# ACMMM2021-Anonymous/video-graph-ssl

Measured on AMD Instinct MI355X. Metric: pretrain_clips_per_sec, higher is better.
Workload: dtype bf16x6 (fp32 tensors; conv products as 6 bf16 MFMAs on hi/mid/lo splits = fp32-grade, fp32 accumulate; everything else fp32)

## Files before the change

__graft_entry__.py:

```python
import importlib
import os
import subprocess
import sys

ROOT = os.path.dirname(os.path.abspath(__file__))
if ROOT not in sys.path:
    sys.path.insert(0, ROOT)
CSRC = os.path.join(ROOT, 'video-graph-ssl_amd', 'csrc')
SOURCES = ['conv3d', 'conv3d_halo', 'conv3d_stem', 'conv3d_pw', 'conv3d_wgrad', 'conv3d_wgrad_ts', 'conv3d_wgrad_stem', 'bn', 'pool', 'misc', 'infonce', 'graph', 'input', 'augment', 'retrieval']


def _hipcc():
    for c in (os.environ.get('HIPCC'), '/opt/rocm/bin/hipcc', 'hipcc'):
        if c and (os.path.isabs(c) and os.path.exists(c) or not os.path.isabs(c)):
            return c
    raise RuntimeError('hipcc not found')


def build(force=False):
    out = os.path.join(ROOT, 'video-graph-ssl_amd', 'libgca_hip.so')
    srcs = [os.path.join(CSRC, s + '.hip') for s in SOURCES]
    deps = srcs + [os.path.join(CSRC, h) for h in ('gca_common.h', 'conv_common.h', 'conv_igemm_host.h', 'conv_halo.h')] + [
                   os.path.join(ROOT, 'include', 'gca_hip.h')]
    stale = force or not os.path.exists(out) or any(os.path.getmtime(d) > os.path.getmtime(out) for d in deps)
    if stale:
        hipcc = _hipcc()
        flags = ['-O3', '--offload-arch=gfx950', '-fPIC', '-std=c++17']
        procs = []
        for s in SOURCES:
            cmd = [hipcc] + flags + ['-c', os.path.join(CSRC, s + '.hip'), '-o', os.path.join(CSRC, s + '.o')]
            procs.append((s, subprocess.Popen(cmd, stdout=subprocess.PIPE, stderr=subprocess.STDOUT)))
        for s, p in procs:
            log = p.communicate()[0].decode()
            if p.returncode != 0:
                raise RuntimeError('hipcc failed on %s.hip:\n%s' % (s, log))
        subprocess.check_call([hipcc, '--offload-arch=gfx950', '-shared', '-fPIC', '-o', out] +
                              [os.path.join(CSRC, s + '.o') for s in SOURCES])
# ... 28 lines not shown
```

include/gca_hip.h:

```cpp
#ifndef GCA_HIP_H
#define GCA_HIP_H

#include <stdint.h>

#ifdef __cplusplus
extern "C" {
#endif

#define GCA_OK 0
#define GCA_EINVAL (-1)
#define GCA_ELAUNCH (-2)

int gca_version(void);

int gca_conv_halo_occupancy(int tm, int tn, int math, int64_t lds_bytes);

int gca_set_conv_math(int mode);
int gca_get_conv_math(void);

typedef struct {
  int32_t N, C, D, H, W;
  int32_t K;
  int32_t kd, kh, kw;
  int32_t sd, sh, sw;
// ... 91 lines not shown
               const float* scale, const float* shift, void* ws, int act_f16, void* stream);
int64_t gca_bn_bwd_consts_elems(int64_t C);
int gca_bn_bwd_sums(const void* dz_in, const void* x, const float* gamma, const float* save_mean, const float* save_invstd,
                    int relu, int64_t N, int64_t C, int64_t SP, float* dgamma, float* dbeta, int64_t z_batch_stride ,
                    const float* scale, const float* shift, float* consts, void* ws, int act_f16, void* stream);

typedef struct {
  int32_t N, C, D, H, W;
  int32_t kd, kh, kw, sd, sh, sw, pd, ph, pw;
  int32_t OD, OH, OW;
} gca_pool_geom;
int gca_maxpool3d_fwd(const gca_pool_geom* g, const void* x, void* y, int32_t* argmax, const float* scale,
                      const float* shift, int act_f16, void* stream);
int gca_maxpool3d_bwd(const gca_pool_geom* g, const void* dy, const int32_t* argmax, void* dx,
                      int accumulate, int act_f16, void* stream);
int gca_avgpool3d_fwd(const gca_pool_geom* g, const float* x, float* y, void* stream);
int gca_avgpool3d_bwd(const gca_pool_geom* g, const float* dy, float* dx, int accumulate, void* stream);
int gca_wavgpool_fwd(const void* x, const float* wt, float norm, int64_t NC, int64_t D, int64_t HW,
                     float* y, int x_f16, void* stream);
int gca_wavgpool_bwd(const float* dy, const float* wt, float norm, int64_t NC, int64_t D, int64_t HW,
                     void* dx, int x_f16, void* stream);

int gca_relu_fwd(const float* x, int64_t n, float* y, void* stream);
int gca_relu_bwd(const float* dy, const float* y, int64_t n, float* dx, void* stream);
int gca_l2norm_fwd(const float* x, int64_t rows, int64_t dim, float eps, float* y, float* inv_norm, void* stream);
int gca_l2norm_bwd(const float* dy, const float* y, const float* inv_norm, int64_t rows, int64_t dim,
                   float* dx, void* stream);
int gca_negcos_fwd_bwd(const float* p, const float* z, int64_t rows, int64_t dim, float scale,
                       float* loss, int accumulate, float* dp, void* stream);

// ... 68 lines not shown
```

video-graph-ssl_amd/_hip.py:

```python
import ctypes as C
import os

import torch

_HERE = os.path.dirname(os.path.abspath(__file__))
LIB_PATH = os.environ.get('GCA_LIB_PATH') or os.path.join(_HERE, 'libgca_hip.so')


class HipLibraryMissing(RuntimeError):
    pass


if not os.path.exists(LIB_PATH):
    raise HipLibraryMissing(
        'libgca_hip.so is not built (%s). Run ./build_hip.sh or __graft_entry__.build(); there is no '
        'CPU fallback for the product path.' % LIB_PATH)
lib = C.CDLL(LIB_PATH)

c_i32, c_i64, c_f32, c_f64, c_vp = C.c_int32, C.c_int64, C.c_float, C.c_double, C.c_void_p


class ConvGeom(C.Structure):
    _fields_ = [(n, c_i32) for n in ('N', 'C', 'D', 'H', 'W', 'K', 'kd', 'kh', 'kw', 'sd', 'sh', 'sw',
                                     'pd', 'ph', 'pw', 'OD', 'OH', 'OW')] + [('x_batch_stride', c_i64)] + \
# ... 30 lines not shown
    'gca_conv_wgrad': (c_i32, [_GP, c_vp, c_vp, c_vp, c_vp, c_i32, c_vp, c_vp]),
    'gca_bias_grad': (c_i32, [c_vp, c_i64, c_i64, c_i64, c_vp, c_i32, c_vp]),
    'gca_bn_stats': (c_i32, [c_vp, c_i64, c_i64, c_i64, c_vp, c_vp, c_vp, c_i32, c_vp]),
    'gca_bn_stats_parts': (c_i64, [c_i64, c_i64, c_i64]),
    'gca_bn_finalize': (c_i32, [c_vp, c_vp, c_i64, c_i64, c_f64, c_vp, c_vp, c_f32, c_f32, c_vp, c_vp, c_vp,
                                c_vp, c_vp, c_vp, c_vp, c_vp]),
    'gca_bn_train_fwd': (c_i32, [c_vp, c_vp, c_i64, c_i64, c_f64, c_vp, c_vp, c_f32, c_f32, c_vp, c_vp, c_vp,
                                 c_vp, c_vp, c_vp, c_vp, c_vp, c_vp, c_i32, c_i64, c_i64, c_vp, c_i64, c_i32, c_vp]),
    'gca_bn_fold_eval': (c_i32, [c_vp, c_vp, c_vp, c_vp, c_f32, c_i64, c_vp, c_vp, c_vp]),
    'gca_bn_apply': (c_i32, [c_vp, c_vp, c_vp, c_vp, c_i32, c_i64, c_i64, c_i64, c_vp, c_i64, c_i32, c_vp]),
    'gca_bn_bwd_ws_bytes': (c_i64, [c_i64, c_i64, c_i64]),
    'gca_bn_bwd': (c_i32, [c_vp, c_vp, c_vp, c_vp, c_vp, c_vp, c_i32, c_i64, c_i64, c_i64, c_vp, c_vp, c_vp,
                           c_vp, c_i32, c_i64, c_vp, c_vp, c_vp, c_i32, c_vp]),
    'gca_maxpool3d_fwd': (c_i32, [_PP, c_vp, c_vp, c_vp, c_vp, c_vp, c_i32, c_vp]),
    'gca_maxpool3d_bwd': (c_i32, [_PP, c_vp, c_vp, c_vp, c_i32, c_i32, c_vp]),
    'gca_avgpool3d_fwd': (c_i32, [_PP, c_vp, c_vp, c_vp]),
    'gca_avgpool3d_bwd': (c_i32, [_PP, c_vp, c_vp, c_i32, c_vp]),
    'gca_wavgpool_fwd': (c_i32, [c_vp, c_vp, c_f32, c_i64, c_i64, c_i64, c_vp, c_i32, c_vp]),
    'gca_wavgpool_bwd': (c_i32, [c_vp, c_vp, c_f32, c_i64, c_i64, c_i64, c_vp, c_i32, c_vp]),
    'gca_relu_fwd': (c_i32, [c_vp, c_i64, c_vp, c_vp]),
    'gca_relu_bwd': (c_i32, [c_vp, c_vp, c_i64, c_vp, c_vp]),
    'gca_l2norm_fwd': (c_i32, [c_vp, c_i64, c_i64, c_f32, c_vp, c_vp, c_vp]),
    'gca_l2norm_bwd': (c_i32, [c_vp, c_vp, c_vp, c_i64, c_i64, c_vp, c_vp]),
    'gca_negcos_fwd_bwd': (c_i32, [c_vp, c_vp, c_i64, c_i64, c_f32, c_vp, c_i32, c_vp, c_vp]),
    'gca_infonce_ws_bytes': (c_i64, [c_i64, c_i64]),
    'gca_moco_logits_fwd': (c_i32, [c_vp, c_vp, c_vp, c_i64, c_i64, c_i64, c_f32, c_vp, c_vp, c_vp, c_vp, c_vp, c_vp, c_vp]),
    'gca_nce_softmax_loss_fwd': (c_i32, [c_vp, c_i64, c_i64, c_vp, c_vp, c_vp, c_vp]),
    'gca_nce_softmax_loss_bwd': (c_i32, [c_vp, c_vp, c_i64, c_i64, c_vp, c_f32, c_vp, c_vp]),
    'gca_moco_logits_bwd': (c_i32, [c_vp, c_vp, c_vp, c_vp, c_f32, c_vp, c_vp, c_i64, c_i64, c_i64, c_f32,
                                    c_i64, c_vp, c_i64, c_vp, c_vp, c_vp, c_vp]),
# ... 95 lines not shown
```

video-graph-ssl_amd/csrc/bn.hip:

```cpp
#include "gca_common.h"

namespace {

constexpr int STAT_CHUNK = 8192;
constexpr int MAX_PARTS = 256;
constexpr long long BN_SMALL_ELEMS = 32768;

__host__ __device__ inline long long stats_parts(long long N, long long C, long long SP) {
  long long p = (N * SP + STAT_CHUNK - 1) / STAT_CHUNK;
  if (p < 1) p = 1;
  if (p > MAX_PARTS) p = MAX_PARTS;
  return p;
}

template <typename T, int MODE, int VEC>
__global__ __launch_bounds__(256) void bn_reduce_kernel(
    const T* __restrict__ a, const T* __restrict__ z, const T* __restrict__ x,
    const float* __restrict__ mean, const float* __restrict__ invstd, int relu,
    long long N, long long C, long long SP, long long zs, int P, float* __restrict__ out0,
    float* __restrict__ out1, const float* __restrict__ scale, const float* __restrict__ shift) {
  typedef gca_act<T> A_;
  __shared__ double sh[4];
  const int c = blockIdx.y, part = blockIdx.x;
  const float rsc = relu == 2 ? scale[c] : 0.f, rsf = relu == 2 ? shift[c] : 0.f;
// ... 494 lines not shown
      if (VEC == 4) {
        A_::st4(dx + xi[u], make_float4(ov[0], ov[VEC > 1 ? 1 : 0], ov[VEC > 2 ? 2 : 0], ov[VEC > 3 ? 3 : 0]));
        if (dres) {
          float4 r = make_float4(dv[u][0], dv[u][VEC > 1 ? 1 : 0], dv[u][VEC > 2 ? 2 : 0], dv[u][VEC > 3 ? 3 : 0]);
          if (dres_acc) { r.x += ro[u].x; r.y += ro[u].y; r.z += ro[u].z; r.w += ro[u].w; }
          A_::st4(dres + xi[u], r);
        }
      } else {
        A_::st(dx + xi[u], ov[0]);
        if (dres) A_::st(dres + xi[u], dres_acc ? ro[u].x + dv[u][0] : dv[u][0]);
      }
    }
  }
}

inline unsigned ew_grid(long long total, int vec) {
  long long b = gca_ceil_div(total, 256LL * vec);
  if (b > 8192) b = 8192;
  if (b < 1) b = 1;
  return (unsigned)b;
}

}

extern "C" int gca_bn_finalize(const float* stat_sum, const float* stat_sq, int64_t P, int64_t C, double count,
                               const float* gamma, const float* beta, float eps, float momentum,
                               float* running_mean, float* running_var, int64_t* num_batches_tracked,
                               float* save_mean, float* save_invstd, float* scale, float* shift, void* stream);

template <typename T>
// ... 122 lines not shown
                         const float* scale, const float* shift, float* consts, void* ws, void* stream) {
  if (!dz_in || !x || !save_mean || !save_invstd || !consts || !ws || N <= 0 || C <= 0 || SP <= 0) return GCA_EINVAL;
  if ((relu != 0 && relu != 2) || (relu == 2 && (!scale || !shift))) return GCA_EINVAL;
  if (z_batch_stride != 0 && z_batch_stride < C * SP) return GCA_EINVAL;
  if (C > 0x7fffffffLL - 32) return GCA_EINVAL;
  const long long zs = z_batch_stride ? z_batch_stride : C * SP;
  const int Cp = (int)gca_bn_consts_stride(C);
  hipStream_t st = (hipStream_t)stream;
  bn_bwd_sums_launch<T>(dz_in, dz_in, x, gamma, save_mean, save_invstd, relu, N, C, SP, zs, dgamma, dbeta, scale, shift, ws,
                        consts, (long long)Cp, st);
  hipLaunchKernelGGL(bn_bwd_consts_kernel, dim3((unsigned)gca_ceil_div(Cp, 256)), dim3(256), 0, st, save_mean, save_invstd,
                     scale, shift, relu, (int)C, Cp, consts);
  return gca_launch_status();
}

extern "C" {

int64_t gca_bn_stats_parts(int64_t N, int64_t C, int64_t SP) { return stats_parts(N, C, SP); }


int gca_bn_finalize(const float* stat_sum, const float* stat_sq, int64_t P, int64_t C, double count,
                    const float* gamma, const float* beta, float eps, float momentum,
                    float* running_mean, float* running_var, int64_t* num_batches_tracked,
                    float* save_mean, float* save_invstd, float* scale, float* shift, void* stream) {
  if (!stat_sum || !stat_sq || P <= 0 || C <= 0 || count <= 0 || !scale || !shift) return GCA_EINVAL;
  hipLaunchKernelGGL(bn_finalize_kernel, dim3((unsigned)C), dim3(256), 0, (hipStream_t)stream, stat_sum, stat_sq,
                     (long long)P, count, gamma, beta, eps, momentum, running_mean, running_var, save_mean,
                     save_invstd, scale, shift, (long long*)num_batches_tracked);
  return gca_launch_status();
}
// ... 74 lines not shown
int64_t gca_bn_bwd_consts_elems(int64_t C) {
  if (C <= 0 || C > 0x7fffffffLL - 32) return GCA_EINVAL;
  return GCA_BN_BWD_CONST_ROWS * gca_bn_consts_stride(C);
}

int gca_bn_bwd_sums(const void* dz_in, const void* x, const float* gamma, const float* save_mean, const float* save_invstd,
                    int relu, int64_t N, int64_t C, int64_t SP, float* dgamma, float* dbeta, int64_t z_batch_stride,
                    const float* scale, const float* shift, float* consts, void* ws, int act_f16, void* stream) {
  if (act_f16)
    return bn_bwd_sums_t<gca_half>((const gca_half*)dz_in, (const gca_half*)x, gamma, save_mean, save_invstd, relu, N, C, SP,
                                   dgamma, dbeta, z_batch_stride, scale, shift, consts, ws, stream);
  return bn_bwd_sums_t<float>((const float*)dz_in, (const float*)x, gamma, save_mean, save_invstd, relu, N, C, SP, dgamma, dbeta,
                              z_batch_stride, scale, shift, consts, ws, stream);
}

}
```

video-graph-ssl_amd/csrc/pool.hip:

```cpp
#include "gca_common.h"
#include <math.h>
#include <cstdlib>

namespace {

struct PoolMagic {
  gca_magic osp, ohw, ow;
  gca_magic sp, hw, w;
  gca_magic sd, sh, sw;
  gca_magic c;
};

template <typename T, int KD, int KH, int KW>
__global__ __launch_bounds__(256) void maxpool3d_fwd_kernel(gca_pool_geom g, PoolMagic q, const T* __restrict__ x,
                                                            T* __restrict__ y, int* __restrict__ argmax,
                                                            unsigned total, const float* __restrict__ scale,
                                                            const float* __restrict__ shift) {
  const unsigned i = blockIdx.x * 256u + threadIdx.x;
  if (i >= total) return;
  const unsigned plane = gca_fdiv(i, q.osp), o = i - plane * q.osp.d;
  float sc = 1.f, sf = 0.f;
  if (scale) { const unsigned c = plane - gca_fdiv(plane, q.c) * q.c.d; sc = scale[c]; sf = shift[c]; }
#define GCA_POOL_VAL(v) (scale ? fmaxf((v) * sc + sf, 0.f) : (v))
  const int od = (int)gca_fdiv(o, q.ohw), r = (int)(o - (unsigned)od * q.ohw.d);
// ... 136 lines not shown
        }
#pragma unroll
    for (int e = 0; e < CD * CH * CW; ++e) acc += (okv[e] && am[e] == s) ? gv[e] : 0.f;
  } else {
    for (int od = od_lo; od <= od_hi; ++od)
      for (int oh = oh_lo; oh <= oh_hi; ++oh)
        for (int ow = ow_lo; ow <= ow_hi; ++ow) {
          const long long o = obase + (long long)od * OHW + oh * g.OW + ow;
          if (argmax[o] == s) acc += (float)dy[o];
        }
  }
  dx[i] = (T)(accumulate ? (float)dx[i] + acc : acc);
}

template <typename T>
__global__ __launch_bounds__(256) void maxpool3d_bwd_brick333s2_kernel(gca_pool_geom g, gca_magic msp, gca_magic mhw, gca_magic mw,
                                                                       const T* __restrict__ dy, const int* __restrict__ argmax,
                                                                       T* __restrict__ dx, unsigned nbricks, int accumulate) {
  const unsigned t = blockIdx.x * 256u + threadIdx.x;
  if (t >= nbricks) return;
  const unsigned plane = gca_fdiv(t, msp), sidx = t - plane * msp.d;
  const int n = (int)gca_fdiv(sidx, mhw), r = (int)(sidx - (unsigned)n * mhw.d);
  const int m = (int)gca_fdiv((unsigned)r, mw), j = r - m * (int)mw.d;
  const bool vd1 = n + 1 < g.OD, vh1 = m + 1 < g.OH, vw2 = 2 * j + 2 < g.OW;
  const unsigned o00 = ((plane * (unsigned)g.OD + (unsigned)n) * (unsigned)g.OH + (unsigned)m) * (unsigned)g.OW + 2u * (unsigned)j;
  const unsigned step_d = vd1 ? (unsigned)(g.OH * g.OW) : 0u, step_h = vh1 ? (unsigned)g.OW : 0u, step_w = vw2 ? 2u : 1u;
  int2 a01[4];
  int a2[4];
  float g0[4], g1[4], g2[4];
#pragma unroll
  for (int c = 0; c < 4; ++c) {
    const unsigned o = o00 + ((c & 2) ? step_d : 0u) + ((c & 1) ? step_h : 0u);
    a01[c] = *reinterpret_cast<const int2*>(argmax + o);
    a2[c] = argmax[o + step_w];
    if (sizeof(T) == 4) {
      const float2 v = *reinterpret_cast<const float2*>(dy + o);
      g0[c] = v.x; g1[c] = v.y;
    } else {
      typedef _Float16 h2 __attribute__((ext_vector_type(2)));
      const h2 v = *reinterpret_cast<const h2*>(dy + o);
      g0[c] = (float)v.x; g1[c] = (float)v.y;
    }
    g2[c] = (float)dy[o + step_w];
  }
  if (!vw2) { a2[0] = a2[1] = a2[2] = a2[3] = -1; }
  if (!vd1) { a01[2] = a01[3] = make_int2(-1, -1); a2[2] = a2[3] = -1; }
  if (!vh1) { a01[1] = a01[3] = make_int2(-1, -1); a2[1] = a2[3] = -1; }
  const unsigned plane_base = plane * (unsigned)(g.D * g.H * g.W);
#pragma unroll
  for (int dd = 0; dd < 2; ++dd)
#pragma unroll
    for (int hh = 0; hh < 2; ++hh) {
      const int d = 2 * n + dd, h = 2 * m + hh;
      if (d >= g.D || h >= g.H) continue;
      const int s0 = (d * g.H + h) * g.W + 4 * j;
      float acc[4] = {0.f, 0.f, 0.f, 0.f};
#pragma unroll
      for (int cd = 0; cd <= dd; ++cd)
#pragma unroll
        for (int ch = 0; ch <= hh; ++ch) {
          const int c = 2 * cd + ch;
          acc[0] += a01[c].x == s0 ? g0[c] : 0.f;
          acc[1] += a01[c].x == s0 + 1 ? g0[c] : 0.f;
          acc[1] += a01[c].y == s0 + 1 ? g1[c] : 0.f;
          acc[2] += a01[c].y == s0 + 2 ? g1[c] : 0.f;
          acc[3] += a01[c].y == s0 + 3 ? g1[c] : 0.f;
          acc[3] += a2[c] == s0 + 3 ? g2[c] : 0.f;
        }
      T* out = dx + (plane_base + (unsigned)s0);
      if (accumulate) {
        const float4 o = gca_act<T>::ld4(out);
        acc[0] += o.x; acc[1] += o.y; acc[2] += o.z; acc[3] += o.w;
      }
      gca_act<T>::st4(out, make_float4(acc[0], acc[1], acc[2], acc[3]));
    }
}

template <typename T>
__global__ __launch_bounds__(256) void wavgpool_fwd_kernel(const T* __restrict__ x, const float* __restrict__ wt,
                                                           float norm, long long NC, int D, int HW,
                                                           float* __restrict__ y) {
  const long long p = (long long)blockIdx.x * 4 + (threadIdx.x >> 6);
  if (p >= NC) return;
// ... 8 lines not shown
  s = gca_wave_sum(s);
  if (lane == 0) y[p] = s * norm;
}

template <typename T>
__global__ __launch_bounds__(256) void wavgpool_bwd_kernel(const float* __restrict__ dy, const float* __restrict__ wt,
                                                           float norm, long long total, int D, int HW,
                                                           T* __restrict__ dx) {
  const long long i = (long long)blockIdx.x * 256 + threadIdx.x;
  if (i >= total) return;
  const long long p = i / ((long long)D * HW);
  const int d = (int)((i / HW) % D);
  dx[i] = (T)(dy[p] * norm * (wt ? wt[d] : 1.f));
}

inline bool pool_ok(const gca_pool_geom* g) {
  if (!g || g->N <= 0 || g->C <= 0 || g->D <= 0 || g->H <= 0 || g->W <= 0) return false;
  if (g->kd <= 0 || g->kh <= 0 || g->kw <= 0 || g->sd <= 0 || g->sh <= 0 || g->sw <= 0) return false;
  if (g->pd < 0 || g->ph < 0 || g->pw < 0 || 2 * g->pd > g->kd || 2 * g->ph > g->kh || 2 * g->pw > g->kw) return false;
  if (g->OD != (g->D + 2 * g->pd - g->kd) / g->sd + 1 || g->OH != (g->H + 2 * g->ph - g->kh) / g->sh + 1 ||
      g->OW != (g->W + 2 * g->pw - g->kw) / g->sw + 1)
    return false;
  return g->OD > 0 && g->OH > 0 && g->OW > 0;
}


__global__ __launch_bounds__(256) void avgpool3d_fwd_kernel(gca_pool_geom g, PoolMagic q, const float* __restrict__ x,
                                                            float* __restrict__ y, unsigned total) {
  const unsigned i = blockIdx.x * 256u + threadIdx.x;
  if (i >= total) return;
  const unsigned plane = gca_fdiv(i, q.osp), o = i - plane * q.osp.d;
  const int od = (int)gca_fdiv(o, q.ohw), r = (int)(o - (unsigned)od * q.ohw.d);
  const int oh = (int)gca_fdiv((unsigned)r, q.ow), ow = r - oh * g.OW;
  const float* xp = x + (long long)plane * ((long long)g.D * g.H * g.W);
  float s = 0.f;
  for (int a = 0; a < g.kd; ++a)
    for (int b = 0; b < g.kh; ++b)
      for (int c = 0; c < g.kw; ++c) s += xp[((od * g.kd + a) * g.H + oh * g.kh + b) * g.W + ow * g.kw + c];
  y[i] = s / (float)(g.kd * g.kh * g.kw);
}
__global__ __launch_bounds__(256) void avgpool3d_bwd_kernel(gca_pool_geom g, PoolMagic q, const float* __restrict__ dy,
// ... 20 lines not shown
}

static PoolMagic pool_magic(const gca_pool_geom* g) {
  PoolMagic q;
  q.osp = gca_make_magic((unsigned)(g->OD * g->OH * g->OW)); q.ohw = gca_make_magic((unsigned)(g->OH * g->OW));
  q.ow = gca_make_magic((unsigned)g->OW);
  q.sp = gca_make_magic((unsigned)(g->D * g->H * g->W)); q.hw = gca_make_magic((unsigned)(g->H * g->W));
  q.w = gca_make_magic((unsigned)g->W);
  q.c = gca_make_magic((unsigned)g->C);
  q.sd = gca_make_magic((unsigned)g->sd); q.sh = gca_make_magic((unsigned)g->sh); q.sw = gca_make_magic((unsigned)g->sw);
  return q;
}

int gca_maxpool3d_fwd(const gca_pool_geom* g, const void* x, void* y, int32_t* argmax, const float* scale,
                      const float* shift, int act_f16, void* stream) {
  if (!pool_ok(g) || !x || !y || ((scale == nullptr) != (shift == nullptr))) return GCA_EINVAL;
  const long long total = (long long)g->N * g->C * g->OD * g->OH * g->OW;
  if (total >= (1LL << 31) || (long long)g->D * g->H * g->W >= (1LL << 31)) return GCA_EINVAL;
  const PoolMagic q = pool_magic(g);
  const dim3 grid((unsigned)gca_ceil_div(total, 256));
  hipStream_t st = (hipStream_t)stream;
#define GCA_POOL_FWD(KD, KH, KW)                                                                                              \
  do {                                                                                                                      \
    if (act_f16)                                                                                                            \
      hipLaunchKernelGGL((maxpool3d_fwd_kernel<gca_half, KD, KH, KW>), grid, dim3(256), 0, st, *g, q, (const gca_half*)x,   \
                         (gca_half*)y, argmax, (unsigned)total, scale, shift);                                              \
    else                                                                                                                    \
      hipLaunchKernelGGL((maxpool3d_fwd_kernel<float, KD, KH, KW>), grid, dim3(256), 0, st, *g, q, (const float*)x,         \
                         (float*)y, argmax, (unsigned)total, scale, shift);                                                 \
  } while (0)
  const size_t esz = act_f16 ? 2 : 4;
  if (g->kd == 3 && g->kh == 3 && g->kw == 3 && g->sd == 2 && g->sh == 2 && g->sw == 2 && g->pd == 1 && g->ph == 1 && g->pw == 1 &&
      g->W % 4 == 0 && ((uintptr_t)x % (4 * esz)) == 0 && ((uintptr_t)y % (2 * esz)) == 0 && ((uintptr_t)argmax % 8) == 0 &&
      pool_tiled_on()) {
    const unsigned npairs = (unsigned)(total / 2);
    const gca_magic psp = gca_make_magic((unsigned)(g->OD * g->OH * (g->OW / 2))), phw = gca_make_magic((unsigned)(g->OH * (g->OW / 2))),
                    pw2 = gca_make_magic((unsigned)(g->OW / 2));
    const dim3 pgrid((unsigned)gca_ceil_div((long long)npairs, 256));
    if (act_f16)
      hipLaunchKernelGGL(maxpool3d_fwd_pair333s2_kernel<gca_half>, pgrid, dim3(256), 0, st, *g, psp, phw, pw2, q.c, (const gca_half*)x,
                         (gca_half*)y, argmax, npairs, scale, shift);
    else
      hipLaunchKernelGGL(maxpool3d_fwd_pair333s2_kernel<float>, pgrid, dim3(256), 0, st, *g, psp, phw, pw2, q.c, (const float*)x,
                         (float*)y, argmax, npairs, scale, shift);
    return gca_launch_status();
  }
  if (g->kd == 3 && g->kh == 3 && g->kw == 3) GCA_POOL_FWD(3, 3, 3);
  else if (g->kd == 1 && g->kh == 3 && g->kw == 3) GCA_POOL_FWD(1, 3, 3);
  else if (g->kd == 2 && g->kh == 2 && g->kw == 2) GCA_POOL_FWD(2, 2, 2);
  else GCA_POOL_FWD(0, 0, 0);
#undef GCA_POOL_FWD
  return gca_launch_status();
}

int gca_maxpool3d_bwd(const gca_pool_geom* g, const void* dy, const int32_t* argmax, void* dx,
                      int accumulate, int act_f16, void* stream) {
  if (!pool_ok(g) || !dy || !argmax || !dx) return GCA_EINVAL;
  const long long total = (long long)g->N * g->C * g->D * g->H * g->W;
  if (total >= (1LL << 31)) return GCA_EINVAL;
  const PoolMagic q = pool_magic(g);
  const dim3 grid((unsigned)gca_ceil_div(total, 256));
  hipStream_t st = (hipStream_t)stream;
  const int cd = (int)gca_ceil_div(g->kd, g->sd), ch = (int)gca_ceil_div(g->kh, g->sh), cw = (int)gca_ceil_div(g->kw, g->sw);
#define GCA_POOL_BWD(CD, CH, CW)                                                                                             \
  do {                                                                                                                     \
    if (act_f16)                                                                                                           \
      hipLaunchKernelGGL((maxpool3d_bwd_kernel<gca_half, CD, CH, CW>), grid, dim3(256), 0, st, *g, q, (const gca_half*)dy, \
                         argmax, (gca_half*)dx, (unsigned)total, accumulate ? 1 : 0);                                      \
    else                                                                                                                   \
      hipLaunchKernelGGL((maxpool3d_bwd_kernel<float, CD, CH, CW>), grid, dim3(256), 0, st, *g, q, (const float*)dy,       \
                         argmax, (float*)dx, (unsigned)total, accumulate ? 1 : 0);                                         \
  } while (0)
  if (g->kd == 3 && g->kh == 3 && g->kw == 3 && g->sd == 2 && g->sh == 2 && g->sw == 2 && g->pd == 1 && g->ph == 1 && g->pw == 1 &&
      g->W % 4 == 0 && ((uintptr_t)dx % (act_f16 ? 8 : 16)) == 0 && ((uintptr_t)dy % (act_f16 ? 4 : 8)) == 0 &&
      ((uintptr_t)argmax % 8) == 0 && pool_tiled_on()) {
    const int d2 = (g->D + 1) / 2, h2 = (g->H + 1) / 2, w4 = g->W / 4;
    const unsigned nbricks = (unsigned)((long long)g->N * g->C * d2 * h2 * w4);
    const gca_magic msp = gca_make_magic((unsigned)(d2 * h2 * w4)), mhw = gca_make_magic((unsigned)(h2 * w4)),
                    mw = gca_make_magic((unsigned)w4);
    const dim3 bgrid((unsigned)gca_ceil_div((long long)nbricks, 256));
    if (act_f16)
      hipLaunchKernelGGL(maxpool3d_bwd_brick333s2_kernel<gca_half>, bgrid, dim3(256), 0, st, *g, msp, mhw, mw, (const gca_half*)dy,
                         argmax, (gca_half*)dx, nbricks, accumulate ? 1 : 0);
    else
      hipLaunchKernelGGL(maxpool3d_bwd_brick333s2_kernel<float>, bgrid, dim3(256), 0, st, *g, msp, mhw, mw, (const float*)dy,
                         argmax, (float*)dx, nbricks, accumulate ? 1 : 0);
    return gca_launch_status();
  }
  if (cd == 2 && ch == 2 && cw == 2) GCA_POOL_BWD(2, 2, 2);
  else if (cd == 1 && ch == 2 && cw == 2) GCA_POOL_BWD(1, 2, 2);
  else if (cd == 3 && ch == 3 && cw == 3) GCA_POOL_BWD(3, 3, 3);
  else if (cd == 1 && ch == 1 && cw == 1) GCA_POOL_BWD(1, 1, 1);
  else GCA_POOL_BWD(0, 0, 0);
#undef GCA_POOL_BWD
  return gca_launch_status();
}

static bool avgpool_ok(const gca_pool_geom* g) {
  return pool_ok(g) && g->sd == g->kd && g->sh == g->kh && g->sw == g->kw && g->pd == 0 && g->ph == 0 && g->pw == 0;
}
int gca_avgpool3d_fwd(const gca_pool_geom* g, const float* x, float* y, void* stream) {
  if (!avgpool_ok(g) || !x || !y) return GCA_EINVAL;
  const long long total = (long long)g->N * g->C * g->OD * g->OH * g->OW;
  if (total >= (1LL << 31) || (long long)g->D * g->H * g->W >= (1LL << 31)) return GCA_EINVAL;
  hipLaunchKernelGGL(avgpool3d_fwd_kernel, dim3((unsigned)gca_ceil_div(total, 256)), dim3(256), 0, (hipStream_t)stream, *g,
                     pool_magic(g), x, y, (unsigned)total);
  return gca_launch_status();
}
int gca_avgpool3d_bwd(const gca_pool_geom* g, const float* dy, float* dx, int accumulate, void* stream) {
  if (!avgpool_ok(g) || !dy || !dx) return GCA_EINVAL;
  const long long total = (long long)g->N * g->C * g->D * g->H * g->W;
  if (total >= (1LL << 31)) return GCA_EINVAL;
  hipLaunchKernelGGL(avgpool3d_bwd_kernel, dim3((unsigned)gca_ceil_div(total, 256)), dim3(256), 0, (hipStream_t)stream, *g,
                     pool_magic(g), dy, dx, (unsigned)total, accumulate ? 1 : 0);
// ... 30 lines not shown
```

video-graph-ssl_amd/engine/layers.py:

```python
import math

import torch
import torch.nn as nn

from . import ops
from . import tape as _tape
from .tape import LazyVar, Var


GRAD_LOG = None


def _grad_of(p):
    if p.grad is None:
        p.grad = torch.zeros_like(p.data)
    if GRAD_LOG is not None:
        GRAD_LOG.append((_tape.CURRENT[0], p))
    return p.grad


class _PackedWeight(object):

    def _init_pack(self):
        self._pack, self._pack_plan, self._prepacked = [None, None], [None, None], [False, False]
# ... 368 lines not shown
        mean, invstd, scale, shift = _bn_scale_shift(bn, ss, sq, N * SP)
    else:
        if xf is not None:
            x, xf = _stored(xv.t), None
        y = ops.conv_fwd(plan, x, wp, None, w_raw=conv.weight.data)
        mean = invstd = None
        scale, shift = ops.bn_fold_eval(bn.weight.data, bn.bias.data, bn.running_mean, bn.running_var, bn.eps)
    pplan = ops.pool_plan(tuple(y.shape), pool.kernel_size, pool.stride, pool.padding)
    p, am = ops.maxpool_fwd(pplan, y, want_argmax=tape.recording, scale=scale, shift=shift)
    pv = Var(p, tape.recording)
    if tape.recording:
        if mean is None:
            raise NotImplementedError('backward through eval-mode BatchNorm is not on the pre-training path')

        def back():
            dz = ops.maxpool_bwd(pplan, pv.grad, am)
            pv.grad = None
            dy = ops.bn_bwd(dz, None, y, bn.weight.data, mean, invstd, 2, N, K, SP, _grad_of(bn.weight), _grad_of(bn.bias),
                            None, False, scale, shift)
            del dz
            ops.conv_wgrad(plan, x, dy, _grad_of(conv.weight), accumulate=True, xf=xf)
            if xv.needs_grad:
                buf, acc = xv.grad_buffer()
                ops.conv_dgrad(plan, dy, conv.packed(plan, 1), buf, acc, w_raw=conv.weight.data)
        tape.record(back)
    return pv


def f_maxpool(tape, pool, xv):
    x = xv.t
    plan = ops.pool_plan(tuple(x.shape), pool.kernel_size, pool.stride, pool.padding)
    y, am = ops.maxpool_fwd(plan, x, want_argmax=tape.recording and xv.needs_grad)
    yv = Var(y, tape.recording)

    def back():
# ... 97 lines not shown
```

video-graph-ssl_amd/engine/ops.py:

```python
import ctypes as C
import functools
import os

import torch

from .. import _hip as H
from .._hip import aptr, is_half, ptr, stream
from . import tune
from .tune import TUNE_HALO, TUNE_PW, TUNE_STEM, TUNE_VEC

F32 = torch.float32
F16 = torch.float16


def _t3(v):
    return (v, v, v) if isinstance(v, int) else tuple(int(a) for a in v)


class _Workspace:

    def __init__(self):
        self.buf = {}
        self.captured = set()
        self.retired = []
# ... 511 lines not shown
def maxpool_fwd(plan, x, want_argmax=True, scale=None, shift=None):
    y = torch.empty(plan.out_shape, dtype=x.dtype, device=x.device)
    am = torch.empty(plan.out_shape, dtype=torch.int32, device=x.device) if want_argmax else None
    H.call('gca_maxpool3d_fwd', plan.gp, aptr(x), aptr(y), ptr(am), ptr(scale), ptr(shift), is_half(x), stream())
    return y, am


def maxpool_bwd(plan, dy, argmax, dx=None, accumulate=False):
    if dx is None:
        dx = torch.empty(plan.in_shape, dtype=dy.dtype, device=dy.device)
        accumulate = False
    H.call('gca_maxpool3d_bwd', plan.gp, aptr(dy), ptr(argmax), aptr(dx), int(accumulate), is_half(dy, dx), stream())
    return dx


def avgpool_fwd(plan, x):
    y = torch.empty(plan.out_shape, dtype=F32, device=x.device)
    H.call('gca_avgpool3d_fwd', plan.gp, ptr(x), ptr(y), stream())
    return y


def avgpool_bwd(plan, dy, dx=None, accumulate=False):
    if dx is None:
        dx = torch.empty(plan.in_shape, dtype=F32, device=dy.device)
        accumulate = False
    H.call('gca_avgpool3d_bwd', plan.gp, ptr(dy), ptr(dx), int(accumulate), stream())
    return dx


def wavgpool_fwd(x, wt, norm):
# ... 256 lines not shown
```

Before: 1690.

## Fuse stem maxpool backward with BN backward via argmax-routed sums and apply

```diff
diff --git a/__graft_entry__.py b/__graft_entry__.py
--- a/__graft_entry__.py
+++ b/__graft_entry__.py
@@ -20,7 +20,7 @@
 def build(force=False):
     out = os.path.join(ROOT, 'video-graph-ssl_amd', 'libgca_hip.so')
     srcs = [os.path.join(CSRC, s + '.hip') for s in SOURCES]
-    deps = srcs + [os.path.join(CSRC, h) for h in ('gca_common.h', 'conv_common.h', 'conv_igemm_host.h', 'conv_halo.h')] + [
+    deps = srcs + [os.path.join(CSRC, h) for h in ('gca_common.h', 'conv_common.h', 'conv_igemm_host.h', 'conv_halo.h', 'pool_brick.h')] + [
                    os.path.join(ROOT, 'include', 'gca_hip.h')]
     stale = force or not os.path.exists(out) or any(os.path.getmtime(d) > os.path.getmtime(out) for d in deps)
     if stale:
diff --git a/include/gca_hip.h b/include/gca_hip.h
--- a/include/gca_hip.h
+++ b/include/gca_hip.h
@@ -129,6 +129,10 @@
                       const float* shift, int act_f16, void* stream);
 int gca_maxpool3d_bwd(const gca_pool_geom* g, const void* dy, const int32_t* argmax, void* dx,
                       int accumulate, int act_f16, void* stream);
+int64_t gca_bn_bwd_pooled_ws_bytes(const gca_pool_geom* g, int any_size);
+int gca_bn_bwd_pooled(const gca_pool_geom* g, const void* dy_pooled, const int32_t* argmax, const void* y, const float* gamma,
+                      const float* save_mean, const float* save_invstd, const float* scale, const float* shift, void* dx,
+                      float* dgamma, float* dbeta, void* ws, int any_size, int act_f16, void* stream);
 int gca_avgpool3d_fwd(const gca_pool_geom* g, const float* x, float* y, void* stream);
 int gca_avgpool3d_bwd(const gca_pool_geom* g, const float* dy, float* dx, int accumulate, void* stream);
 int gca_wavgpool_fwd(const void* x, const float* wt, float norm, int64_t NC, int64_t D, int64_t HW,
diff --git a/video-graph-ssl_amd/_hip.py b/video-graph-ssl_amd/_hip.py
--- a/video-graph-ssl_amd/_hip.py
+++ b/video-graph-ssl_amd/_hip.py
@@ -68,6 +68,8 @@
                            c_vp, c_i32, c_i64, c_vp, c_vp, c_vp, c_i32, c_vp]),
     'gca_maxpool3d_fwd': (c_i32, [_PP, c_vp, c_vp, c_vp, c_vp, c_vp, c_i32, c_vp]),
     'gca_maxpool3d_bwd': (c_i32, [_PP, c_vp, c_vp, c_vp, c_i32, c_i32, c_vp]),
+    'gca_bn_bwd_pooled_ws_bytes': (c_i64, [_PP, c_i32]),
+    'gca_bn_bwd_pooled': (c_i32, [_PP, c_vp, c_vp, c_vp, c_vp, c_vp, c_vp, c_vp, c_vp, c_vp, c_vp, c_vp, c_vp, c_i32, c_i32, c_vp]),
     'gca_avgpool3d_fwd': (c_i32, [_PP, c_vp, c_vp, c_vp]),
     'gca_avgpool3d_bwd': (c_i32, [_PP, c_vp, c_vp, c_i32, c_vp]),
     'gca_wavgpool_fwd': (c_i32, [c_vp, c_vp, c_f32, c_i64, c_i64, c_i64, c_vp, c_i32, c_vp]),
diff --git a/video-graph-ssl_amd/csrc/bn.hip b/video-graph-ssl_amd/csrc/bn.hip
--- a/video-graph-ssl_amd/csrc/bn.hip
+++ b/video-graph-ssl_amd/csrc/bn.hip
@@ -1,10 +1,19 @@
 #include "gca_common.h"
+#include "pool_brick.h"
 
 namespace {
 
 constexpr int STAT_CHUNK = 8192;
 constexpr int MAX_PARTS = 256;
 constexpr long long BN_SMALL_ELEMS = 32768;
+constexpr int POOLED_CHUNK = 2048;
+
+__host__ __device__ inline long long pooled_parts(long long N, long long OSP) {
+  long long p = (N * OSP + POOLED_CHUNK - 1) / POOLED_CHUNK;
+  if (p < 1) p = 1;
+  if (p > MAX_PARTS) p = MAX_PARTS;
+  return p;
+}
 
 __host__ __device__ inline long long stats_parts(long long N, long long C, long long SP) {
   long long p = (N * SP + STAT_CHUNK - 1) / STAT_CHUNK;
@@ -532,6 +541,109 @@
   }
 }
 
+template <typename T>
+__global__ __launch_bounds__(256) void bn_bwd_pooled_sums333s2_kernel(
+    const T* __restrict__ gp, const int* __restrict__ argmax, const T* __restrict__ x,
+    const float* __restrict__ mean, const float* __restrict__ invstd, const float* __restrict__ scale,
+    const float* __restrict__ shift, unsigned M , unsigned C, gca_magic osp, unsigned SP, int P,
+    float* __restrict__ out0, float* __restrict__ out1) {
+  typedef gca_act<T> A_;
+  __shared__ double sh[4];
+  const unsigned c = blockIdx.y, part = blockIdx.x;
+  const float rsc = scale[c], rsf = shift[c], mu = mean[c], is = invstd[c];
+  unsigned per = (M + (unsigned)P - 1) / (unsigned)P;
+  per = (per + 1) & ~1u;
+  const unsigned lo = part * per;
+  const unsigned hi = lo + per < M ? lo + per : M;
+  double s0 = 0.0, s1 = 0.0;
+  constexpr int UF = 4;
+  for (unsigned i0 = lo + 2u * threadIdx.x; i0 < hi; i0 += 512u * UF) {
+    int2 a[UF];
+    float g0[UF], g1[UF], y0[UF], y1[UF];
+    unsigned xb[UF];
+#pragma unroll
+    for (int u = 0; u < UF; ++u) {
+      const unsigned i = min(i0 + 512u * u, hi - 2u);
+      const unsigned n = gca_fdiv(i, osp), o = i - n * osp.d;
+      const unsigned pi = (n * C + c) * osp.d + o;
+      xb[u] = (n * C + c) * SP;
+      a[u] = *reinterpret_cast<const int2*>(argmax + pi);
+      if (sizeof(T) == 4) {
+        const float2 v = *reinterpret_cast<const float2*>(gp + pi);
+        g0[u] = v.x; g1[u] = v.y;
+      } else {
+        typedef _Float16 h2 __attribute__((ext_vector_type(2)));
+        const h2 v = *reinterpret_cast<const h2*>(gp + pi);
+        g0[u] = (float)v.x; g1[u] = (float)v.y;
+      }
+    }
+#pragma unroll
+    for (int u = 0; u < UF; ++u) {
+      y0[u] = A_::ld(x + (xb[u] + min((unsigned)max(a[u].x, 0), SP - 1u)));
+      y1[u] = A_::ld(x + (xb[u] + min((unsigned)max(a[u].y, 0), SP - 1u)));
+    }
+#pragma unroll
+    for (int u = 0; u < UF; ++u) {
+      if (i0 + 512u * u >= hi) break;
+      float d0 = g0[u], d1 = g1[u];
+      if (!(y0[u] * rsc + rsf > 0.f)) d0 = 0.f;
+      if (!(y1[u] * rsc + rsf > 0.f)) d1 = 0.f;
+      s0 += (double)d0; s1 += (double)d0 * (double)((y0[u] - mu) * is);
+      s0 += (double)d1; s1 += (double)d1 * (double)((y1[u] - mu) * is);
+    }
+  }
+  s0 = gca_block_sum256_d(s0, sh);
+  s1 = gca_block_sum256_d(s1, sh);
+  if (threadIdx.x == 0) {
+    out0[(long long)c * P + part] = (float)s0;
+    out1[(long long)c * P + part] = (float)s1;
+  }
+}
+
+template <typename T>
+__global__ __launch_bounds__(256) void bn_bwd_apply_routed333s2_kernel(
+    gca_pool_geom g, gca_brick_magic q, gca_magic cm, const T* __restrict__ gp, const int* __restrict__ argmax,
+    const T* __restrict__ x, const float* __restrict__ mean, const float* __restrict__ invstd, const float* __restrict__ coef,
+    const float* __restrict__ scale, const float* __restrict__ shift, T* __restrict__ dx, unsigned nbricks) {
+  typedef gca_act<T> A_;
+  const unsigned t = blockIdx.x * 256u + threadIdx.x;
+  if (t >= nbricks) return;
+  gca_pool_brick<T> b;
+  b.load(g, q, t, gp, argmax);
+  const unsigned plane_base = b.plane * (unsigned)(g.D * g.H * g.W);
+  float4 xq[4];
+#pragma unroll
+  for (int e = 0; e < 4; ++e) {
+    const int d = min(2 * b.n + (e >> 1), g.D - 1), h = min(2 * b.m + (e & 1), g.H - 1);
+    xq[e] = A_::ld4(x + (plane_base + (unsigned)((d * g.H + h) * g.W + 4 * b.j)));
+  }
+  const unsigned c = b.plane - gca_fdiv(b.plane, cm) * cm.d;
+  const unsigned C = cm.d;
+  const float A = coef[c], B = coef[C + c], Cc = coef[2 * C + c], mu = mean[c], is = invstd[c];
+  const float rsc = scale[c], rsf = shift[c];
+  b.mask();
+#pragma unroll
+  for (int dd = 0; dd < 2; ++dd)
+#pragma unroll
+    for (int hh = 0; hh < 2; ++hh) {
+      const int d = 2 * b.n + dd, h = 2 * b.m + hh;
+      if (d >= g.D || h >= g.H) continue;
+      const int s0 = (d * g.H + h) * g.W + 4 * b.j;
+      float dz[4];
+      b.quad(dd, hh, s0, dz);
+      const float4 xv = xq[2 * dd + hh];
+      const float xe[4] = {xv.x, xv.y, xv.z, xv.w};
+      float o[4];
+#pragma unroll
+      for (int e = 0; e < 4; ++e) {
+        float dv = (float)(T)dz[e];
+        if (!(xe[e] * rsc + rsf > 0.f)) dv = 0.f;
+        o[e] = A * (dv - B - (xe[e] - mu) * is * Cc);
+      }
+      A_::st4(dx + (plane_base + (unsigned)s0), make_float4(o[0], o[1], o[2], o[3]));
+    }
+}
+
 inline unsigned ew_grid(long long total, int vec) {
   long long b = gca_ceil_div(total, 256LL * vec);
   if (b > 8192) b = 8192;
@@ -684,6 +796,39 @@
   return gca_launch_status();
 }
 
+static bool bn_bwd_pooled_geom_ok(const gca_pool_geom* g, int any_size) {
+  if (!gca_pool_geom_ok(g) || !gca_pool_brick_geom(g)) return false;
+  const long long SP = (long long)g->D * g->H * g->W;
+  if ((long long)g->N * g->C * SP >= (1LL << 31)) return false;
+  return any_size || (long long)g->N * SP > BN_SMALL_ELEMS;
+}
+
+template <typename T>
+static int bn_bwd_pooled_t(const gca_pool_geom* g, const T* gp, const int32_t* argmax, const T* y, const float* gamma,
+                           const float* save_mean, const float* save_invstd, const float* scale, const float* shift, T* dx,
+                           float* dgamma, float* dbeta, void* ws, int any_size, void* stream) {
+  if (!bn_bwd_pooled_geom_ok(g, any_size)) return GCA_EINVAL;
+  if (!gp || !argmax || !y || !save_mean || !save_invstd || !scale || !shift || !dx || !ws) return GCA_EINVAL;
+  if (((uintptr_t)y | (uintptr_t)dx) % (4 * sizeof(T)) || (uintptr_t)gp % (2 * sizeof(T)) || (uintptr_t)argmax % 8 ||
+      (uintptr_t)ws % 4)
+    return GCA_EINVAL;
+  hipStream_t st = (hipStream_t)stream;
+  const long long N = g->N, C = g->C, SP = (long long)g->D * g->H * g->W, OSP = (long long)g->OD * g->OH * g->OW;
+  const int P = (int)pooled_parts(N, OSP);
+  float* p0 = reinterpret_cast<float*>(ws);
+  float* p1 = p0 + C * P;
+  float* coef = p1 + C * P;
+  hipLaunchKernelGGL(bn_bwd_pooled_sums333s2_kernel<T>, dim3((unsigned)P, (unsigned)C), dim3(256), 0, st, gp, argmax, y, save_mean,
+                     save_invstd, scale, shift, (unsigned)(N * OSP), (unsigned)C, gca_make_magic((unsigned)OSP), (unsigned)SP, P, p0, p1);
+  hipLaunchKernelGGL(bn_bwd_finalize_kernel, dim3((unsigned)C), dim3(256), 0, st, p0, p1, P, (double)N * (double)SP, gamma,
+                     save_invstd, dgamma, dbeta, coef, C);
+  const unsigned nbricks = (unsigned)gca_pool_bricks(g);
+  hipLaunchKernelGGL(bn_bwd_apply_routed333s2_kernel<T>, dim3((unsigned)gca_ceil_div((long long)nbricks, 256)), dim3(256), 0, st, *g,
+                     gca_make_brick_magic(g), gca_make_magic((unsigned)C), gp, argmax, y, save_mean, save_invstd, coef, scale, shift,
+                     dx, nbricks);
+  return gca_launch_status();
+}
+
 extern "C" {
 
 int64_t gca_bn_stats_parts(int64_t N, int64_t C, int64_t SP) { return stats_parts(N, C, SP); }
@@ -788,4 +933,20 @@
                               z_batch_stride, scale, shift, consts, ws, stream);
 }
 
-}
+int64_t gca_bn_bwd_pooled_ws_bytes(const gca_pool_geom* g, int any_size) {
+  if (!bn_bwd_pooled_geom_ok(g, any_size)) return GCA_EINVAL;
+  const long long C = g->C;
+  return (int64_t)sizeof(float) * (2 * C * pooled_parts(g->N, (long long)g->OD * g->OH * g->OW) + 3 * C);
+}
+
+int gca_bn_bwd_pooled(const gca_pool_geom* g, const void* dy_pooled, const int32_t* argmax, const void* y, const float* gamma,
+                      const float* save_mean, const float* save_invstd, const float* scale, const float* shift, void* dx,
+                      float* dgamma, float* dbeta, void* ws, int any_size, int act_f16, void* stream) {
+  if (act_f16)
+    return bn_bwd_pooled_t<gca_half>(g, (const gca_half*)dy_pooled, argmax, (const gca_half*)y, gamma, save_mean, save_invstd,
+                                     scale, shift, (gca_half*)dx, dgamma, dbeta, ws, any_size, stream);
+  return bn_bwd_pooled_t<float>(g, (const float*)dy_pooled, argmax, (const float*)y, gamma, save_mean, save_invstd, scale, shift,
+                                (float*)dx, dgamma, dbeta, ws, any_size, stream);
+}
+
+}
diff --git a/video-graph-ssl_amd/csrc/pool.hip b/video-graph-ssl_amd/csrc/pool.hip
--- a/video-graph-ssl_amd/csrc/pool.hip
+++ b/video-graph-ssl_amd/csrc/pool.hip
@@ -1,4 +1,5 @@
 #include "gca_common.h"
+#include "pool_brick.h"
 #include <math.h>
 #include <cstdlib>
 
@@ -174,59 +175,24 @@
 }
 
 template <typename T>
-__global__ __launch_bounds__(256) void maxpool3d_bwd_brick333s2_kernel(gca_pool_geom g, gca_magic msp, gca_magic mhw, gca_magic mw,
+__global__ __launch_bounds__(256) void maxpool3d_bwd_brick333s2_kernel(gca_pool_geom g, gca_brick_magic q,
                                                                        const T* __restrict__ dy, const int* __restrict__ argmax,
                                                                        T* __restrict__ dx, unsigned nbricks, int accumulate) {
   const unsigned t = blockIdx.x * 256u + threadIdx.x;
   if (t >= nbricks) return;
-  const unsigned plane = gca_fdiv(t, msp), sidx = t - plane * msp.d;
-  const int n = (int)gca_fdiv(sidx, mhw), r = (int)(sidx - (unsigned)n * mhw.d);
-  const int m = (int)gca_fdiv((unsigned)r, mw), j = r - m * (int)mw.d;
-  const bool vd1 = n + 1 < g.OD, vh1 = m + 1 < g.OH, vw2 = 2 * j + 2 < g.OW;
-  const unsigned o00 = ((plane * (unsigned)g.OD + (unsigned)n) * (unsigned)g.OH + (unsigned)m) * (unsigned)g.OW + 2u * (unsigned)j;
-  const unsigned step_d = vd1 ? (unsigned)(g.OH * g.OW) : 0u, step_h = vh1 ? (unsigned)g.OW : 0u, step_w = vw2 ? 2u : 1u;
-  int2 a01[4];
-  int a2[4];
-  float g0[4], g1[4], g2[4];
-#pragma unroll
-  for (int c = 0; c < 4; ++c) {
-    const unsigned o = o00 + ((c & 2) ? step_d : 0u) + ((c & 1) ? step_h : 0u);
-    a01[c] = *reinterpret_cast<const int2*>(argmax + o);
-    a2[c] = argmax[o + step_w];
-    if (sizeof(T) == 4) {
-      const float2 v = *reinterpret_cast<const float2*>(dy + o);
-      g0[c] = v.x; g1[c] = v.y;
-    } else {
-      typedef _Float16 h2 __attribute__((ext_vector_type(2)));
-      const h2 v = *reinterpret_cast<const h2*>(dy + o);
-      g0[c] = (float)v.x; g1[c] = (float)v.y;
-    }
-    g2[c] = (float)dy[o + step_w];
-  }
-  if (!vw2) { a2[0] = a2[1] = a2[2] = a2[3] = -1; }
-  if (!vd1) { a01[2] = a01[3] = make_int2(-1, -1); a2[2] = a2[3] = -1; }
-  if (!vh1) { a01[1] = a01[3] = make_int2(-1, -1); a2[1] = a2[3] = -1; }
-  const unsigned plane_base = plane * (unsigned)(g.D * g.H * g.W);
+  gca_pool_brick<T> b;
+  b.load(g, q, t, dy, argmax);
+  b.mask();
+  const unsigned plane_base = b.plane * (unsigned)(g.D * g.H * g.W);
 #pragma unroll
   for (int dd = 0; dd < 2; ++dd)
 #pragma unroll
     for (int hh = 0; hh < 2; ++hh) {
-      const int d = 2 * n + dd, h = 2 * m + hh;
+      const int d = 2 * b.n + dd, h = 2 * b.m + hh;
       if (d >= g.D || h >= g.H) continue;
-      const int s0 = (d * g.H + h) * g.W + 4 * j;
-      float acc[4] = {0.f, 0.f, 0.f, 0.f};
-#pragma unroll
-      for (int cd = 0; cd <= dd; ++cd)
-#pragma unroll
-        for (int ch = 0; ch <= hh; ++ch) {
-          const int c = 2 * cd + ch;
-          acc[0] += a01[c].x == s0 ? g0[c] : 0.f;
-          acc[1] += a01[c].x == s0 + 1 ? g0[c] : 0.f;
-          acc[1] += a01[c].y == s0 + 1 ? g1[c] : 0.f;
-          acc[2] += a01[c].y == s0 + 2 ? g1[c] : 0.f;
-          acc[3] += a01[c].y == s0 + 3 ? g1[c] : 0.f;
-          acc[3] += a2[c] == s0 + 3 ? g2[c] : 0.f;
-        }
+      const int s0 = (d * g.H + h) * g.W + 4 * b.j;
+      float acc[4];
+      b.quad(dd, hh, s0, acc);
       T* out = dx + (plane_base + (unsigned)s0);
       if (accumulate) {
         const float4 o = gca_act<T>::ld4(out);
@@ -265,17 +231,6 @@
   dx[i] = (T)(dy[p] * norm * (wt ? wt[d] : 1.f));
 }
 
-inline bool pool_ok(const gca_pool_geom* g) {
-  if (!g || g->N <= 0 || g->C <= 0 || g->D <= 0 || g->H <= 0 || g->W <= 0) return false;
-  if (g->kd <= 0 || g->kh <= 0 || g->kw <= 0 || g->sd <= 0 || g->sh <= 0 || g->sw <= 0) return false;
-  if (g->pd < 0 || g->ph < 0 || g->pw < 0 || 2 * g->pd > g->kd || 2 * g->ph > g->kh || 2 * g->pw > g->kw) return false;
-  if (g->OD != (g->D + 2 * g->pd - g->kd) / g->sd + 1 || g->OH != (g->H + 2 * g->ph - g->kh) / g->sh + 1 ||
-      g->OW != (g->W + 2 * g->pw - g->kw) / g->sw + 1)
-    return false;
-  return g->OD > 0 && g->OH > 0 && g->OW > 0;
-}
-
-
 __global__ __launch_bounds__(256) void avgpool3d_fwd_kernel(gca_pool_geom g, PoolMagic q, const float* __restrict__ x,
                                                             float* __restrict__ y, unsigned total) {
   const unsigned i = blockIdx.x * 256u + threadIdx.x;
@@ -326,7 +281,7 @@
 
 int gca_maxpool3d_fwd(const gca_pool_geom* g, const void* x, void* y, int32_t* argmax, const float* scale,
                       const float* shift, int act_f16, void* stream) {
-  if (!pool_ok(g) || !x || !y || ((scale == nullptr) != (shift == nullptr))) return GCA_EINVAL;
+  if (!gca_pool_geom_ok(g) || !x || !y || ((scale == nullptr) != (shift == nullptr))) return GCA_EINVAL;
   const long long total = (long long)g->N * g->C * g->OD * g->OH * g->OW;
   if (total >= (1LL << 31) || (long long)g->D * g->H * g->W >= (1LL << 31)) return GCA_EINVAL;
   const PoolMagic q = pool_magic(g);
@@ -342,8 +297,7 @@
                          (float*)y, argmax, (unsigned)total, scale, shift);                                                 \
   } while (0)
   const size_t esz = act_f16 ? 2 : 4;
-  if (g->kd == 3 && g->kh == 3 && g->kw == 3 && g->sd == 2 && g->sh == 2 && g->sw == 2 && g->pd == 1 && g->ph == 1 && g->pw == 1 &&
-      g->W % 4 == 0 && ((uintptr_t)x % (4 * esz)) == 0 && ((uintptr_t)y % (2 * esz)) == 0 && ((uintptr_t)argmax % 8) == 0 &&
+  if (gca_pool_brick_geom(g) && ((uintptr_t)x % (4 * esz)) == 0 && ((uintptr_t)y % (2 * esz)) == 0 && ((uintptr_t)argmax % 8) == 0 &&
       pool_tiled_on()) {
     const unsigned npairs = (unsigned)(total / 2);
     const gca_magic psp = gca_make_magic((unsigned)(g->OD * g->OH * (g->OW / 2))), phw = gca_make_magic((unsigned)(g->OH * (g->OW / 2))),
@@ -367,7 +321,7 @@
 
 int gca_maxpool3d_bwd(const gca_pool_geom* g, const void* dy, const int32_t* argmax, void* dx,
                       int accumulate, int act_f16, void* stream) {
-  if (!pool_ok(g) || !dy || !argmax || !dx) return GCA_EINVAL;
+  if (!gca_pool_geom_ok(g) || !dy || !argmax || !dx) return GCA_EINVAL;
   const long long total = (long long)g->N * g->C * g->D * g->H * g->W;
   if (total >= (1LL << 31)) return GCA_EINVAL;
   const PoolMagic q = pool_magic(g);
@@ -383,19 +337,16 @@
       hipLaunchKernelGGL((maxpool3d_bwd_kernel<float, CD, CH, CW>), grid, dim3(256), 0, st, *g, q, (const float*)dy,       \
                          argmax, (float*)dx, (unsigned)total, accumulate ? 1 : 0);                                         \
   } while (0)
-  if (g->kd == 3 && g->kh == 3 && g->kw == 3 && g->sd == 2 && g->sh == 2 && g->sw == 2 && g->pd == 1 && g->ph == 1 && g->pw == 1 &&
-      g->W % 4 == 0 && ((uintptr_t)dx % (act_f16 ? 8 : 16)) == 0 && ((uintptr_t)dy % (act_f16 ? 4 : 8)) == 0 &&
+  if (gca_pool_brick_geom(g) && ((uintptr_t)dx % (act_f16 ? 8 : 16)) == 0 && ((uintptr_t)dy % (act_f16 ? 4 : 8)) == 0 &&
       ((uintptr_t)argmax % 8) == 0 && pool_tiled_on()) {
-    const int d2 = (g->D + 1) / 2, h2 = (g->H + 1) / 2, w4 = g->W / 4;
-    const unsigned nbricks = (unsigned)((long long)g->N * g->C * d2 * h2 * w4);
-    const gca_magic msp = gca_make_magic((unsigned)(d2 * h2 * w4)), mhw = gca_make_magic((unsigned)(h2 * w4)),
-                    mw = gca_make_magic((unsigned)w4);
+    const unsigned nbricks = (unsigned)gca_pool_bricks(g);
+    const gca_brick_magic bq = gca_make_brick_magic(g);
     const dim3 bgrid((unsigned)gca_ceil_div((long long)nbricks, 256));
     if (act_f16)
-      hipLaunchKernelGGL(maxpool3d_bwd_brick333s2_kernel<gca_half>, bgrid, dim3(256), 0, st, *g, msp, mhw, mw, (const gca_half*)dy,
+      hipLaunchKernelGGL(maxpool3d_bwd_brick333s2_kernel<gca_half>, bgrid, dim3(256), 0, st, *g, bq, (const gca_half*)dy,
                          argmax, (gca_half*)dx, nbricks, accumulate ? 1 : 0);
     else
-      hipLaunchKernelGGL(maxpool3d_bwd_brick333s2_kernel<float>, bgrid, dim3(256), 0, st, *g, msp, mhw, mw, (const float*)dy,
+      hipLaunchKernelGGL(maxpool3d_bwd_brick333s2_kernel<float>, bgrid, dim3(256), 0, st, *g, bq, (const float*)dy,
                          argmax, (float*)dx, nbricks, accumulate ? 1 : 0);
     return gca_launch_status();
   }
@@ -409,7 +360,7 @@
 }
 
 static bool avgpool_ok(const gca_pool_geom* g) {
-  return pool_ok(g) && g->sd == g->kd && g->sh == g->kh && g->sw == g->kw && g->pd == 0 && g->ph == 0 && g->pw == 0;
+  return gca_pool_geom_ok(g) && g->sd == g->kd && g->sh == g->kh && g->sw == g->kw && g->pd == 0 && g->ph == 0 && g->pw == 0;
 }
 int gca_avgpool3d_fwd(const gca_pool_geom* g, const float* x, float* y, void* stream) {
   if (!avgpool_ok(g) || !x || !y) return GCA_EINVAL;
diff --git a/video-graph-ssl_amd/csrc/pool_brick.h b/video-graph-ssl_amd/csrc/pool_brick.h
--- /dev/null
+++ b/video-graph-ssl_amd/csrc/pool_brick.h
@@ -0,0 +1,90 @@
+#pragma once
+#include "gca_common.h"
+
+static inline bool gca_pool_geom_ok(const gca_pool_geom* g) {
+  if (!g || g->N <= 0 || g->C <= 0 || g->D <= 0 || g->H <= 0 || g->W <= 0) return false;
+  if (g->kd <= 0 || g->kh <= 0 || g->kw <= 0 || g->sd <= 0 || g->sh <= 0 || g->sw <= 0) return false;
+  if (g->pd < 0 || g->ph < 0 || g->pw < 0 || 2 * g->pd > g->kd || 2 * g->ph > g->kh || 2 * g->pw > g->kw) return false;
+  if (g->OD != (g->D + 2 * g->pd - g->kd) / g->sd + 1 || g->OH != (g->H + 2 * g->ph - g->kh) / g->sh + 1 ||
+      g->OW != (g->W + 2 * g->pw - g->kw) / g->sw + 1)
+    return false;
+  return g->OD > 0 && g->OH > 0 && g->OW > 0;
+}
+
+static inline bool gca_pool_brick_geom(const gca_pool_geom* g) {
+  return g->kd == 3 && g->kh == 3 && g->kw == 3 && g->sd == 2 && g->sh == 2 && g->sw == 2 && g->pd == 1 && g->ph == 1 && g->pw == 1 &&
+         g->W % 4 == 0;
+}
+
+struct gca_brick_magic { gca_magic sp, hw, w; };
+static inline long long gca_pool_bricks(const gca_pool_geom* g) {
+  return (long long)g->N * g->C * ((g->D + 1) / 2) * ((g->H + 1) / 2) * (g->W / 4);
+}
+static inline gca_brick_magic gca_make_brick_magic(const gca_pool_geom* g) {
+  const int d2 = (g->D + 1) / 2, h2 = (g->H + 1) / 2, w4 = g->W / 4;
+  gca_brick_magic q;
+  q.sp = gca_make_magic((unsigned)(d2 * h2 * w4)); q.hw = gca_make_magic((unsigned)(h2 * w4)); q.w = gca_make_magic((unsigned)w4);
+  return q;
+}
+
+#ifdef __HIPCC__
+template <typename T>
+struct gca_pool_brick {
+  unsigned plane;
+  int n, m, j;
+  bool vd1, vh1, vw2;
+  int2 a01[4];
+  int a2[4];
+  float g0[4], g1[4], g2[4];
+
+  __device__ __forceinline__ void load(const gca_pool_geom& g, const gca_brick_magic& q, unsigned t, const T* __restrict__ dy,
+                                       const int* __restrict__ argmax) {
+    plane = gca_fdiv(t, q.sp);
+    const unsigned sidx = t - plane * q.sp.d;
+    n = (int)gca_fdiv(sidx, q.hw);
+    const int r = (int)(sidx - (unsigned)n * q.hw.d);
+    m = (int)gca_fdiv((unsigned)r, q.w); j = r - m * (int)q.w.d;
+    vd1 = n + 1 < g.OD; vh1 = m + 1 < g.OH; vw2 = 2 * j + 2 < g.OW;
+    const unsigned o00 = ((plane * (unsigned)g.OD + (unsigned)n) * (unsigned)g.OH + (unsigned)m) * (unsigned)g.OW + 2u * (unsigned)j;
+    const unsigned step_d = vd1 ? (unsigned)(g.OH * g.OW) : 0u, step_h = vh1 ? (unsigned)g.OW : 0u, step_w = vw2 ? 2u : 1u;
+#pragma unroll
+    for (int c = 0; c < 4; ++c) {
+      const unsigned o = o00 + ((c & 2) ? step_d : 0u) + ((c & 1) ? step_h : 0u);
+      a01[c] = *reinterpret_cast<const int2*>(argmax + o);
+      a2[c] = argmax[o + step_w];
+      if (sizeof(T) == 4) {
+        const float2 v = *reinterpret_cast<const float2*>(dy + o);
+        g0[c] = v.x; g1[c] = v.y;
+      } else {
+        typedef _Float16 h2 __attribute__((ext_vector_type(2)));
+        const h2 v = *reinterpret_cast<const h2*>(dy + o);
+        g0[c] = (float)v.x; g1[c] = (float)v.y;
+      }
+      g2[c] = (float)dy[o + step_w];
+    }
+  }
+
+  __device__ __forceinline__ void mask() {
+    if (!vw2) { a2[0] = a2[1] = a2[2] = a2[3] = -1; }
+    if (!vd1) { a01[2] = a01[3] = make_int2(-1, -1); a2[2] = a2[3] = -1; }
+    if (!vh1) { a01[1] = a01[3] = make_int2(-1, -1); a2[1] = a2[3] = -1; }
+  }
+
+  __device__ __forceinline__ void quad(int dd, int hh, int s0, float (&acc)[4]) const {
+    acc[0] = acc[1] = acc[2] = acc[3] = 0.f;
+#pragma unroll
+    for (int cd = 0; cd < 2; ++cd)
+#pragma unroll
+      for (int ch = 0; ch < 2; ++ch) {
+        if (cd > dd || ch > hh) continue;
+        const int c = 2 * cd + ch;
+        acc[0] += a01[c].x == s0 ? g0[c] : 0.f;
+        acc[1] += a01[c].x == s0 + 1 ? g0[c] : 0.f;
+        acc[1] += a01[c].y == s0 + 1 ? g1[c] : 0.f;
+        acc[2] += a01[c].y == s0 + 2 ? g1[c] : 0.f;
+        acc[3] += a01[c].y == s0 + 3 ? g1[c] : 0.f;
+        acc[3] += a2[c] == s0 + 3 ? g2[c] : 0.f;
+      }
+  }
+};
+#endif
diff --git a/video-graph-ssl_amd/engine/layers.py b/video-graph-ssl_amd/engine/layers.py
--- a/video-graph-ssl_amd/engine/layers.py
+++ b/video-graph-ssl_amd/engine/layers.py
@@ -406,11 +406,16 @@
             raise NotImplementedError('backward through eval-mode BatchNorm is not on the pre-training path')
 
         def back():
-            dz = ops.maxpool_bwd(pplan, pv.grad, am)
+            dy = None
+            if ops.STEM_POOL_BWD:
+                dy = ops.bn_bwd_pooled(pplan, pv.grad, am, y, bn.weight.data, mean, invstd, scale, shift,
+                                       _grad_of(bn.weight), _grad_of(bn.bias))
+            if dy is None:
+                dz = ops.maxpool_bwd(pplan, pv.grad, am)
+                dy = ops.bn_bwd(dz, None, y, bn.weight.data, mean, invstd, 2, N, K, SP, _grad_of(bn.weight), _grad_of(bn.bias),
+                                None, False, scale, shift)
+                del dz
             pv.grad = None
-            dy = ops.bn_bwd(dz, None, y, bn.weight.data, mean, invstd, 2, N, K, SP, _grad_of(bn.weight), _grad_of(bn.bias),
-                            None, False, scale, shift)
-            del dz
             ops.conv_wgrad(plan, x, dy, _grad_of(conv.weight), accumulate=True, xf=xf)
             if xv.needs_grad:
                 buf, acc = xv.grad_buffer()
diff --git a/video-graph-ssl_amd/engine/ops.py b/video-graph-ssl_amd/engine/ops.py
--- a/video-graph-ssl_amd/engine/ops.py
+++ b/video-graph-ssl_amd/engine/ops.py
@@ -549,6 +549,23 @@
     return dx
 
 
+STEM_POOL_BWD = os.environ.get('GCA_STEM_POOL_BWD', '1') != '0'
+
+
+def bn_bwd_pooled(plan, dp, argmax, y, gamma, mean, invstd, scale, shift, dgamma, dbeta, any_size=False):
+    nbytes = H.lib.gca_bn_bwd_pooled_ws_bytes(plan.gp, int(any_size))
+    if nbytes < 0:
+        return None
+    dy = torch.empty_like(y)
+    ws = WS.get(nbytes, y.device)
+    rc = H.lib.gca_bn_bwd_pooled(plan.gp, aptr(dp), ptr(argmax), aptr(y), ptr(gamma), ptr(mean), ptr(invstd), ptr(scale), ptr(shift),
+                                 aptr(dy), ptr(dgamma), ptr(dbeta), ptr(ws), int(any_size), is_half(dp, y), stream())
+    if rc == -1:
+        return None
+    H.check(rc, 'gca_bn_bwd_pooled')
+    return dy
+
+
 def avgpool_fwd(plan, x):
     y = torch.empty(plan.out_shape, dtype=F32, device=x.device)
     H.call('gca_avgpool3d_fwd', plan.gp, ptr(x), ptr(y), stream())
```

Measured after the change: 1716 (median of 6 runs). About the same (+1.6%).
